# hcherkaoui/pybold

Measured on AMD Instinct MI355X. Metric: voxel-iterations/sec, higher is better.
Workload: dtype f16x2-split operands (22 bit), f32 accumulate, f64 iterate

## Files before the change

include/pybold_hip.h:

```cpp
#ifndef PYBOLD_HIP_H
#define PYBOLD_HIP_H

#include <stdint.h>

#ifdef __cplusplus
extern "C" {
#endif

#define PB_OK 0
#define PB_ERR_INVALID (-1)
#define PB_ERR_HIP (-2)

#define PB_FLAG_FORCE_GENERIC 1u
#define PB_FLAG_FORCE_FAST 2u
#define PB_FLAG_NO_PAIR 4u
#define PB_FLAG_FORCE_PAIR 8u
#define PB_FLAG_FORCE_WIDE 16u
#define PB_FLAG_DIRECT_FIR 64u
#define PB_FLAG_ONE_STREAM 128u
#define PB_FLAG_COLD_START 256u
#define PB_FLAG_NO_CERT 512u
#define PB_FLAG_CERT_NO_RESOLVE 2048u
#define PB_FLAG_FORCE_MFMA 16384u
#define PB_FLAG_NO_RHO_GUARD 32768u
#define PB_FLAG_FORCE_MFMA2 65536u
#define PB_FLAG_NO_MFMA 8192u
#define PB_FLAG_FORCE_CERT 1024u
#define PB_FLAG_NO_PARTITION 4096u
#define PB_FLAG_ONLY_DENSE 131072u
#define PB_FLAG_ONLY_SPARSE 262144u
#define PB_FLAG_NO_ILL_GUARD 524288u
#define PB_FLAG_PP_SPLIT 1048576u
#define PB_FLAG_LONG_HRF 2097152u
enum { PB_FLAG_MFMA_DENSE_TILES = 4194304 };
enum { PB_FLAG_GROUPED_SPLIT = 8388608 };
#define PB_FLAG_ONE_LAUNCH 32u

#define PB_STOP_NONE 0
#define PB_STOP_LOOPS 1
#define PB_STOP_WINDOW 2

int pb_version(void);

int pb_init(void);

const char* pb_last_error(void);

int pb_fista_has_fast_path(int N, int K);

int pb_fista_which_kernel(int N, int K, int P, int with_cost_trace, int stop_mode, int wind);

int pb_fista_plan(int N, int K, int P, int stop_mode, int wind, int* n_main, int* main_form,
                  int* tail_form);
int pb_fista_plan_ex(int N, int K, int P, int stop_mode, int wind, unsigned flags, int* n_main,
                     int* main_form, int* tail_form);

int pb_fista_solve(const float* y_dev, int64_t ldy, int y_rep,
                   double* w_dev, int64_t ldw, int P, int N,
                   const double* taps_host, const double* taps_dev, int K,
                   double step, double lbda, const double* lbda_dev,
                   const double* betas_dev, int n_iter,
                   float* J_dev, int64_t ldj,
                   int stop_mode, double tol, int wind, int32_t* n_done_dev,
                   unsigned flags, void* stream);

int64_t pb_fista_work_len(int P, int y_rep);
#define PB_CAND_COUNT 10
int pb_fista_list_plan(int kind, int n, int n_max, int has_pair, int has_wide, int one_stream, int has_mfma2,
// ... 222 lines not shown
```

pybold_amd/_lib.py:

```python
import ctypes
import os

_HERE = os.path.dirname(os.path.abspath(__file__))
LIB_PATH = os.environ.get("PYBOLD_HIP_LIB") or os.path.join(_HERE, "libpybold_hip.so")

PB_FLAG_FORCE_GENERIC = 1
PB_FLAG_FORCE_FAST = 2
PB_FLAG_NO_PAIR = 4
PB_FLAG_FORCE_PAIR = 8
PB_FLAG_FORCE_WIDE = 16
PB_FLAG_ONE_LAUNCH = 32
PB_FLAG_DIRECT_FIR = 64
PB_FLAG_ONE_STREAM = 128
PB_FLAG_COLD_START = 256
PB_FLAG_NO_CERT = 512
PB_FLAG_FORCE_CERT = 1024
PB_FLAG_CERT_NO_RESOLVE = 2048
PB_FLAG_NO_PARTITION = 4096
PB_FLAG_NO_MFMA = 8192
PB_FLAG_FORCE_MFMA = 16384
PB_FLAG_NO_RHO_GUARD = 32768
PB_FLAG_FORCE_MFMA2 = 65536
PB_FLAG_ONLY_DENSE = 131072
PB_FLAG_ONLY_SPARSE = 262144
PB_FLAG_NO_ILL_GUARD = 524288
PB_FLAG_PP_SPLIT = 1048576
PB_FLAG_MFMA_DENSE_TILES = 4194304
PB_FLAG_LONG_HRF = 2097152
PB_FLAG_GROUPED_SPLIT = 8388608
PB_PATH_DENSE_RATIO = 0.19
PB_STOP_NONE = 0
PB_STOP_LOOPS = 1
PB_STOP_WINDOW = 2

_c_int = ctypes.c_int
_c_i64 = ctypes.c_int64
_c_dbl = ctypes.c_double
_ptr = ctypes.c_void_p

_SOLVE_D = [
    _ptr, _c_i64, _c_int,
    _ptr, _c_i64, _c_int, _c_int,
    _ptr, _ptr, _c_int,
    _c_dbl, _c_dbl, _ptr,
    _ptr, _c_int,
    _ptr, _c_i64,
    _c_int, _c_dbl, _c_int, _ptr,
    ctypes.c_uint, _ptr]
_SOLVE_PP_D = [
    _ptr, _c_i64, _c_int,
    _ptr, _c_i64, _c_int, _c_int,
    _ptr, _c_i64, _c_int, _ptr,
    _c_dbl, _ptr,
    _ptr, _c_int,
    _ptr, _c_i64,
    _c_int, _c_dbl, _c_int, _ptr,
    ctypes.c_uint, _ptr]
_AUTO_LBDA_D = [
    _ptr, _c_i64, _ptr, _c_i64, _c_int, _c_int, _c_int,
    _ptr, _c_int, _c_dbl, _ptr, _ptr,
    _c_int, _c_dbl, _c_int, _c_int, _c_int, _c_int,
    _ptr, _ptr, _ptr, _c_i64,
# ... 176 lines not shown
```

pybold_amd/csrc/capi.hip:

```cpp
#include "../../include/pybold_hip.h"

#include <cstdarg>
#include <cstdlib>
#include <cstdio>
#include <cmath>
#include <cstring>
#include <map>
#include <mutex>

#include "fista_fast.h"
#include "generic.h"
#include "launch_fast.h"
#include "fista_pair.h"
#include "fista_pair_ffa.h"
#include "fista_exact.h"
#include "fista_exact_split.h"
#include "fista_auto.h"
#include "fista_exact_pp.h"
#include "fista_exact_split_pp.h"
#include "blind.h"
#include "fista_mfma.h"
#include "fista_mfma_sparse.h"
#include "fista_mfma_grouped.h"
#include "grouped.h"
#include "fista_mfma2.h"
#include "fista_mfma4.h"
#include "fista_mfma_split_grouped.h"
#include "path.h"
#include "dispatch.h"

namespace {

thread_local char g_err[512] = "";

int fail(int code, const char* fmt, ...) {
  va_list ap;
  va_start(ap, fmt);
  vsnprintf(g_err, sizeof(g_err), fmt, ap);
  va_end(ap);
  return code;
}

int check_launch(const char* what) {
  hipError_t e = hipGetLastError();
  if (e != hipSuccess) return fail(PB_ERR_HIP, "%s: %s", what, hipGetErrorString(e));
  g_err[0] = 0;
  return PB_OK;
}

constexpr int LDS_DOUBLES_MAX = 20000;
inline int64_t gen_lds_doubles(int N, int K, int stop_mode, int wind) {
  return 3 * (int64_t)N + K + 2 * pb::GEN_WAVES + (stop_mode == PB_STOP_WINDOW ? (int64_t)wind * N : 0);
}

inline int auto_outer_chunk(int form, int V, int nb_sub_iter) {
// ... 21 lines not shown
struct SideStream {
  hipStream_t stream = nullptr;
  hipEvent_t fork = nullptr, join = nullptr;
  bool ok = false;
};
std::mutex g_side_mutex;

SideStream* side_stream_locked() {
  static std::map<int, SideStream> per_dev;
  int dev = 0;
  if (hipGetDevice(&dev) != hipSuccess) return nullptr;
  SideStream& ss = per_dev[dev];
  if (!ss.ok && ss.stream == nullptr) {
    int least = 0, greatest = 0;
    if (hipDeviceGetStreamPriorityRange(&least, &greatest) != hipSuccess) { least = greatest = 0; (void)hipGetLastError(); }
    if (hipStreamCreateWithPriority(&ss.stream, hipStreamNonBlocking, greatest) == hipSuccess &&
        hipEventCreateWithFlags(&ss.fork, hipEventDisableTiming) == hipSuccess &&
        hipEventCreateWithFlags(&ss.join, hipEventDisableTiming) == hipSuccess)
      ss.ok = true;
    else
      (void)hipGetLastError();
  }
  return ss.ok ? &ss : nullptr;
}

bool stream_is_capturing(hipStream_t st) {
  hipStreamCaptureStatus cs = hipStreamCaptureStatusNone;
  if (hipStreamIsCapturing(st, &cs) != hipSuccess) {
    (void)hipGetLastError();
    return true;
  }
  return cs != hipStreamCaptureStatusNone;
}
struct WorkLayout { int64_t ranges, lmax, total; };
WorkLayout work_layout(int P, int V) {
  const int64_t nblk = ((int64_t)P + pb::PATH_PER_BLOCK - 1) / pb::PATH_PER_BLOCK;
  WorkLayout w;
  w.ranges = ((int64_t)P + 2 + 2 * nblk + 8 + 1) & ~(int64_t)1;
  w.lmax = w.ranges + 3 * 2 * pb::CAND_COUNT + 4;
  w.total = w.lmax + 2 * (int64_t)V + 8;
  return w;
}
int32_t* own_workspace(void* stream, int64_t need, int64_t* len) {
  static std::mutex mu;
  static std::map<std::pair<int, void*>, std::pair<int32_t*, int64_t>> cache;
  int dev = 0;
  if (hipGetDevice(&dev) != hipSuccess) { (void)hipGetLastError(); return nullptr; }
  std::lock_guard<std::mutex> lock(mu);
  auto& e = cache[std::make_pair(dev, stream)];
  if (e.second < need) {
    int32_t* fresh = nullptr;
    const int64_t want = need + need / 4;
    if (hipMalloc((void**)&fresh, (size_t)want * sizeof(int32_t)) != hipSuccess) { (void)hipGetLastError(); return nullptr; }
    e.first = fresh;
    e.second = want;
  }
  *len = e.second;
  return e.first;
}

template <int KIND>
int launch_op(const double* x, int64_t ldx, double* out, int64_t ldo, int V, int n_src, int n_dst,
              const double* taps, int K, void* stream, const char* name) {
  if (V < 0 || n_src < 1 || n_dst < 1 || K < 0)
    return fail(PB_ERR_INVALID, "%s: bad size (V=%d n_src=%d n_dst=%d K=%d)", name, V, n_src, n_dst, K);
  if (ldx < n_src || ldo < n_dst) return fail(PB_ERR_INVALID, "%s: leading dimension too small", name);
  const int nmax = n_src > n_dst ? n_src : n_dst;
  if (2 * (int64_t)nmax + K + 8 > LDS_DOUBLES_MAX)
    return fail(PB_ERR_INVALID, "%s: row of %d with %d taps exceeds LDS", name, nmax, K);
  if (V == 0) return PB_OK;
  if (!x || !out || (K > 0 && !taps)) return fail(PB_ERR_INVALID, "%s: NULL pointer", name);
  const size_t lds = (size_t)(2 * nmax + K + 8) * sizeof(double);
// ... 278 lines not shown
}

struct PartitionSpecs { pb::PlanSpec dense, sparse, flagged; };
PartitionSpecs partition_specs(const Route& r, int N, bool one_stream) {
  const double slots = wave_slots();
  const int pair = r.has_pair ? 1 : 0, wide = r.has_wide ? 1 : 0, os = one_stream ? 1 : 0;
  if (r.path == PATH_PART_SHORT)
    return {{1, pair, wide, 0, os, r.has_mfma2 ? 1 : 0, r.beside_chunks, slots}, {2, pair, wide, 0, os, 0, 0, slots}, {2, 0, wide, 0, 1, 0, 0, slots}};
  PartitionSpecs s{{3, 0, 0, 0, 1, 1, 0, slots}, {4, pair, 0, 0, 1, 0, 0, slots}, {4, 0, 0, 0, 1, 0, 0, slots}};
  if (N > 640) {
    s.dense.pass_mult = 2;
    s.dense.rem_num16 = MFMA4_MIN_R_NUM;
  }
  s.dense.backup_form = s.sparse.backup_form = s.flagged.backup_form = r.backup_wide ? FORM_WIDE : FORM_FAST1;
  s.sparse.min_pair = SPLIT_MIN_P;
  return s;
}
bool list_has_form(const Route& r, int form, int list) {
  const bool lng = r.path == PATH_PART_LONG;
  if (form == FORM_MFMA) return list <= 1 && r.mfma != nullptr;
  if (form == FORM_MFMA2) return list <= 1 && (lng || r.has_mfma2);
  if (list == 1) return false;
  if (form == FORM_PAIR) return list != 3 && r.has_pair;
  if (form == FORM_WIDE) return lng ? r.backup_wide : r.has_wide;
  return !lng || !r.backup_wide;
}
int cand_bound(const Route& r, int c, int P) {
  if (r.path == PATH_PART_SHORT) return pb::cand_max_slots(c, P, wave_slots());
  return (c == pb::CAND_MFMA2 || c == pb::CAND_PAIR0 || c == pb::CAND_FAST0 || c == pb::CAND_WIDE) ? P : 0;
}

template <class LF>
int solve_list(const Route& r, const pb::FistaArgs& a, const LF& lf, hipStream_t user, Side& side, const int32_t* work_dev,
               const int32_t* ranges, int list, bool exact_rule) {
  pb::FistaArgs b = a;
  b.perm = work_dev;
  b.n_dense = work_dev + a.P;
  b.perm_side = list == 3 ? 3 : 1;
  int rc = PB_OK;
  for (int c = 0; c < pb::CAND_COUNT && rc == PB_OK; ++c) {
    const int form = pb::cand_form(c);
    if (!list_has_form(r, form, list) || (pb::cand_side(c) && !side.ss)) continue;
    if ((c == pb::CAND_PAIR1 || c == pb::CAND_FAST1) && !side.ss) continue;
    b.grid_slots = cand_bound(r, c, a.P);
    if (b.grid_slots <= 0) continue;
    if (c >= pb::CAND_FIRST_AFTER_FORK && side.ss) rc = side.fork(user, lf.name);
    if (rc != PB_OK) break;
    b.range = ranges + 2 * c;
    rc = launch(lf, form, b, (pb::cand_side(c) && side.ss) ? side.ss->stream : user, exact_rule);
  }
  const int rj = side.join(user, lf.name);
  return rj != PB_OK ? rj : rc;
}

void launch_lmax_pass(const pb::FistaArgs& a, int V_series, const double* taps_host, double* lm, double gamma_f64, double gamma_vec,
                      hipStream_t st) {
  const int N = a.N, K = a.K;
  pb::LmaxTaps lt;
  double run = 0.0, csum = 0.0;
  for (int k = 0; k < pb::LMAX_KT; ++k) lt.h[k] = k < K ? (float)taps_host[k] : 0.0f;
  for (int t = 0; t < N; ++t) { if (t < K) run += taps_host[t]; csum += std::fabs(run); }
  const double unit = csum / std::sqrt((double)N);
  const float f64_bound = gamma_f64 > 0.0 ? (float)(gamma_f64 * unit) : 0.0f, vec_bound = gamma_vec > 0.0 ? (float)(gamma_vec * unit) : 0.0f;
  const dim3 grid((unsigned)((V_series + 3) / 4)), block(256);
  if (N <= 320) hipLaunchKernelGGL((pb::lmax_wave_kernel<5>), grid, block, 4 * (64 * 5 + pb::LMAX_KT) * sizeof(float), st, a.y, a.ldy, V_series, N, lt, K, lm, f64_bound, vec_bound);
  else if (N <= 640) hipLaunchKernelGGL((pb::lmax_wave_kernel<10>), grid, block, 4 * (64 * 10 + pb::LMAX_KT) * sizeof(float), st, a.y, a.ldy, V_series, N, lt, K, lm, f64_bound, vec_bound);
  else hipLaunchKernelGGL((pb::lmax_wave_kernel<21>), grid, block, 4 * (64 * 21 + pb::LMAX_KT) * sizeof(float), st, a.y, a.ldy, V_series, N, lt, K, lm, f64_bound, vec_bound);
}

int launch_partition(const pb::ClassPred& cp, int P, int32_t* work_dev, const pb::PlanSpec& front, const pb::PlanSpec& back,
                     int32_t* rg_front, int32_t* rg_back, int32_t* rg_ill, const char* what, hipStream_t st) {
  const int nblk = (P + pb::PATH_PER_BLOCK - 1) / pb::PATH_PER_BLOCK;
  hipLaunchKernelGGL(pb::path_count_kernel, dim3(nblk), dim3(pb::PATH_THREADS), 0, st, cp, P, work_dev);
  hipLaunchKernelGGL(pb::path_scan_kernel, dim3(1), dim3(pb::PATH_THREADS), 0, st, P, nblk, work_dev, front, back, rg_front, rg_back, rg_ill);
  hipLaunchKernelGGL(pb::path_scatter_kernel, dim3(nblk), dim3(pb::PATH_THREADS), 0, st, cp, P, work_dev);
  return check_launch(what);
}

void launch_generic(const pb::FistaArgs& a, const double* taps_dev, int K, int wind, bool with_j, bool f64, int grid, hipStream_t st) {
  void (*const kernel)(pb::FistaArgs, const double*, int, int) =
      !f64 ? (with_j ? pb::fista_generic_kernel<true> : pb::fista_generic_kernel<false>)
           : (with_j ? pb::fista_generic_kernel<true, true> : pb::fista_generic_kernel<false, true>);
  hipLaunchKernelGGL(kernel, dim3(grid), dim3(pb::GEN_THREADS), (size_t)gen_lds_doubles(a.N, K, a.stop_mode, wind) * sizeof(double), st,
                     a, taps_dev, K, wind);
}

template <class LF>
int run_partition(const Route& r, const pb::FistaArgs& a, const LF& lf, hipStream_t user, const double* taps_host,
                  const double* taps_dev, unsigned flags, double dense_ratio, int32_t* work_dev) {
  const int P = a.P, N = a.N, K = a.K, V_series = (P + a.y_rep - 1) / a.y_rep;
  const bool one_stream = r.path == PATH_PART_LONG || (flags & PB_FLAG_ONE_STREAM) != 0 || stream_is_capturing(user);
  const PartitionSpecs sp = partition_specs(r, N, one_stream);
  const WorkLayout wl = work_layout(P, V_series);
  const ExactEntry* ill_exact = pick_f64_default(N, K, a.stop_mode, a.wind, true);
  const bool ill_generic = !ill_exact && taps_dev && gen_lds_doubles(N, K, a.stop_mode, a.wind) <= LDS_DOUBLES_MAX;
  const bool guard = !(flags & PB_FLAG_NO_ILL_GUARD);
  double* lmax = reinterpret_cast<double*>(work_dev + wl.lmax);
  launch_lmax_pass(a, V_series, taps_host, lmax, (guard && (ill_exact || ill_generic)) ? PART_GAMMA_F64 : 0.0,
                   guard ? part_gamma_matrix_pipe(N, K) : 0.0, user);
  int32_t* rg_dense = work_dev + wl.ranges;
  int32_t* rg_sparse = rg_dense + 2 * pb::CAND_COUNT;
  int32_t* rg_flag = rg_sparse + 2 * pb::CAND_COUNT;
  int32_t* rg_ill = rg_flag + 2 * pb::CAND_COUNT;
  const double ratio = (r.path == PATH_PART_SHORT && !r.mfma) ? 0.0
                       : dense_ratio > 0.0 ? dense_ratio
                       : N > 640 ? PB_PATH_DENSE_RATIO_LONGER : (N > MFMA1_NMAX ? PB_PATH_DENSE_RATIO_LONG : PB_PATH_DENSE_RATIO);
  pb::PlanSpec front = sp.dense;
  front.merged = 1;
  int rc = launch_partition(pb::ClassPred{a.lbda_vec, a.lbda, lmax, a.y_rep, ratio, nullptr}, P, work_dev, front, sp.sparse, rg_dense,
                            rg_sparse, rg_ill, "partition", user);
  if (rc != PB_OK) return rc;
  Side side;
  if (!one_stream) side.take();
  const bool only_dense = (flags & PB_FLAG_ONLY_DENSE) != 0, only_sparse = (flags & PB_FLAG_ONLY_SPARSE) != 0;
  rc = solve_list(r, a, lf, user, side, work_dev, rg_dense, only_dense ? 1 : (only_sparse ? 2 : 0), false);
  if (rc != PB_OK || only_dense || only_sparse) return rc;
  if (ill_exact || ill_generic) {
    pb::FistaArgs b = a;
    b.perm = work_dev;
    b.perm_side = 1;
    b.range = rg_ill;
    if (ill_exact) {
      b.grid_slots = P;
      if (ill_exact->fn(b, taps_host, K, a.J != nullptr, a.stop_mode, user) != 0)
        return fail(PB_ERR_INVALID, "%s: float64 kernel rejected the launch (ill-conditioned series)", lf.name);
    } else {
      launch_generic(b, taps_dev, K, a.wind, a.J != nullptr, false, P < 2048 ? P : 2048, user);
    }
    rc = check_launch("float64 kernel (ill-conditioned series)");
    if (rc != PB_OK) return rc;
  }
  const pb::PlanSpec none{0, 0, 0, 0, 1, 0, 0, sp.dense.slots};
  rc = launch_partition(pb::ClassPred{nullptr, 0.0, nullptr, 1, 0.0, a.n_done}, P, work_dev, sp.flagged, none, rg_flag, nullptr, nullptr,
                        "partition(handed back)", user);
  if (rc != PB_OK) return rc;
  side.ss = nullptr;
  return solve_list(r, a, lf, user, side, work_dev, rg_flag, 3, true);
}

int outputs_impl(const double* w_dev, int64_t ldw, int P, int N, const double* taps_dev, int64_t ldt, int K, double* z_dev,
                 int64_t ldz, double* x_dev, int64_t ldx, void* stream, bool pp, const char* name) {
  if (P < 0 || N < 1 || K < 1 || ldw < N || (pp && ldt < K) || (z_dev && ldz < N) || (x_dev && ldx < N))
    return fail(PB_ERR_INVALID, "%s: bad size", name);
  if (2 * (int64_t)N + K + 8 > LDS_DOUBLES_MAX) return fail(PB_ERR_INVALID, "%s: N=%d K=%d exceeds LDS", name, N, K);
  if (P == 0 || (!z_dev && !x_dev)) return PB_OK;
  if (!w_dev || !taps_dev) return fail(PB_ERR_INVALID, "%s: NULL pointer", name);
  const size_t lds = (size_t)(2 * N + K + 8) * sizeof(double);
  hipLaunchKernelGGL(pb::outputs_kernel, dim3(P), dim3(pb::GEN_THREADS), lds, (hipStream_t)stream,
// ... 68 lines not shown

static int solve_impl(const float* y_dev, int64_t ldy, int y_rep, double* w_dev, int64_t ldw, int P,
                      int N, const double* taps_host, const double* taps_dev, int K, double step,
                      double lbda,
                      const double* lbda_dev, const double* betas_dev, int n_iter, float* J_dev,
                      int64_t ldj, int stop_mode, double tol, int wind, int32_t* n_done_dev,
                      unsigned flags, void* stream, const double* lmax_dev, double dense_ratio,
                      int32_t* work_dev, int64_t work_len) {
  if (P < 0 || N < 1 || K < 1 || n_iter < 0 || y_rep < 1)
    return fail(PB_ERR_INVALID, "pb_fista_solve: bad size (P=%d N=%d K=%d n_iter=%d y_rep=%d)", P,
                N, K, n_iter, y_rep);
  if (P > 0 && (!y_dev || !w_dev || !taps_host || (n_iter > 0 && !betas_dev)))
    return fail(PB_ERR_INVALID, "pb_fista_solve: NULL pointer");
  if (P > (1 << 25)) return fail(PB_ERR_INVALID, "pb_fista_solve: more than 2^25 problems per launch");
  if (ldy < N || ldw < N) return fail(PB_ERR_INVALID, "pb_fista_solve: leading dimension < N");
  if (J_dev && ldj < n_iter) return fail(PB_ERR_INVALID, "pb_fista_solve: ldj < n_iter");
  if (!(step > 0.0)) return fail(PB_ERR_INVALID, "pb_fista_solve: step must be positive");
  if (!lbda_dev && lbda < 0.0) return fail(PB_ERR_INVALID, "pb_fista_solve: negative lbda (float64 entry point only)");
  if (stop_mode < PB_STOP_NONE || stop_mode > PB_STOP_WINDOW)
    return fail(PB_ERR_INVALID, "pb_fista_solve: unknown stop_mode %d", stop_mode);
  if (stop_mode == PB_STOP_WINDOW && wind < 2)
    return fail(PB_ERR_INVALID, "pb_fista_solve: wind must be >= 2");
  if (P == 0) return PB_OK;

  pb::FistaArgs a = fista_args(P, N, K, n_iter, y_rep, ldy, w_dev, ldw, step, lbda, lbda_dev, betas_dev, stop_mode, tol,
                               n_done_dev, flags);
  a.y = y_dev; a.J = J_dev; a.ldj = ldj; a.wind = wind;
#ifdef PB_DEVELOPMENT
  if (const char* yb = getenv("PB_MFMA_YBITS")) {
    const int v = atoi(yb);
    if (v >= 8 && v <= 15) a.ybits = v;
  }
#endif
  const int V_series = (P + y_rep - 1) / y_rep;
  const bool workspace = work_dev && work_len >= work_layout(P, V_series).total && !((flags & PB_FLAG_FORCE_MFMA) && !lmax_dev);
  const Route r = route(Call{N, K, P, stop_mode, wind, flags, J_dev != nullptr, lbda_dev != nullptr, n_done_dev != nullptr,
                             tol * (double)n_iter, taps_dev != nullptr, workspace, false});
  const hipStream_t user = (hipStream_t)stream;
  const HostTapsForms lf{r, "pb_fista_solve", taps_host, K, stop_mode, J_dev != nullptr, (flags & PB_FLAG_DIRECT_FIR) != 0};
  if (r.path == PATH_PART_LONG || r.path == PATH_PART_SHORT)
    return run_partition(r, a, lf, user, taps_host, taps_dev, flags, dense_ratio, work_dev);
  if (r.path != PATH_GENERIC) return run_in_place(r, a, lf, user, flags);
  if (flags & PB_FLAG_FORCE_FAST)
    return fail(PB_ERR_INVALID, "pb_fista_solve: no register-resident kernel for N=%d K=%d stop=%d",
                N, K, stop_mode);
  if (!taps_dev) return fail(PB_ERR_INVALID, "pb_fista_solve: taps_dev required for the generic kernel");
  if (gen_lds_doubles(N, K, stop_mode, wind) > LDS_DOUBLES_MAX)
    return fail(PB_ERR_INVALID, "pb_fista_solve: N=%d K=%d wind=%d exceeds LDS", N, K, wind);
  launch_generic(a, taps_dev, K, wind, J_dev != nullptr, false, P, user);
  return check_launch("fista_generic_kernel");
}

int pb_fista_list_plan(int kind, int n, int n_max, int has_pair, int has_wide, int one_stream, int has_mfma2,
                       int beside_chunks, int32_t* ranges, int32_t* bounds) {
  if (kind < 1 || kind > 3 || n < 0 || n_max < n) return fail(PB_ERR_INVALID, "pb_fista_list_plan: bad argument");
  Piece pc[pb::MAX_PIECES];
  int npc = 0;
  const double slots = wave_slots();
  if (n > 0 && kind == 1) npc = pb::plan_pieces_mfma(n, has_pair != 0, has_wide != 0, false, one_stream != 0, has_mfma2 != 0, beside_chunks, slots, pc);
  else if (n > 0 && kind == 2) npc = pb::plan_pieces(n, has_pair != 0, has_wide != 0, false, one_stream != 0, slots, pc);
  else if (kind == 3 && n_max > 0)
    npc = pb::plan_partitioned(n, n_max, has_pair != 0, has_wide != 0, one_stream != 0, has_mfma2 != 0, beside_chunks, slots, pc);
  int32_t rg[2 * pb::CAND_COUNT];
  const int rc = pb::plan_to_candidates(pc, npc, rg);
  for (int c = 0; c < pb::CAND_COUNT; ++c) {
    if (ranges) { ranges[2 * c] = rg[2 * c]; ranges[2 * c + 1] = rg[2 * c + 1]; }
// ... 806 lines not shown
```

pybold_amd/csrc/path.h:

```cpp
#pragma once
#include <hip/hip_runtime.h>
#include <stdint.h>

#include "plan.h"

namespace pb {

constexpr int PATH_THREADS = 256, PATH_PER_THREAD = 16, PATH_PER_BLOCK = PATH_THREADS * PATH_PER_THREAD;

struct ClassPred {
  const double* lbda;
  double lbda_s;
  const double* lmax;
  int y_rep;
  double ratio;
  const int32_t* n_done;
};

__device__ __forceinline__ int path_class(const ClassPred& c, int p) {
  if (c.n_done) return c.n_done[p] < 0 ? 0 : 1;
  const double lm = c.lmax[p / c.y_rep];
  if (lm < 0.0) return 2;
  const double lb = c.lbda ? c.lbda[p] : c.lbda_s;
  return lb < c.ratio * lm ? 0 : 1;
// ... 4 lines not shown
__global__ __launch_bounds__(PATH_THREADS) void path_count_kernel(ClassPred cp, int P, int32_t* work) {
  __shared__ int part[2][PATH_THREADS / 64];
  const int p0 = blockIdx.x * PATH_PER_BLOCK + threadIdx.x * PATH_PER_THREAD;
  int c = 0, ci = 0;
  for (int i = 0; i < PATH_PER_THREAD; ++i) {
    if (p0 + i >= P) break;
    const int k = path_class(cp, p0 + i);
    c += k == 0;
    ci += k == 2;
  }
  for (int o = 32; o > 0; o >>= 1) { c += __shfl_xor(c, o, 64); ci += __shfl_xor(ci, o, 64); }
  if ((threadIdx.x & 63) == 0) { part[0][threadIdx.x >> 6] = c; part[1][threadIdx.x >> 6] = ci; }
  __syncthreads();
  if (threadIdx.x == 0) {
    work[P + 1 + blockIdx.x] = part[0][0] + part[0][1] + part[0][2] + part[0][3];
    work[P + 1 + gridDim.x + blockIdx.x] = part[1][0] + part[1][1] + part[1][2] + part[1][3];
  }
}

struct PlanSpec {
  int kind;
  int has_pair, has_wide, one_launch, one_stream, has_mfma2, beside_chunks;
  double slots;
  int backup_form = FORM_WIDE;
  int min_pair = 1024;
  int pass_mult = 4;
  int rem_num16 = 5;
  int merged = 0;
};
__device__ __forceinline__ void plan_list(const PlanSpec& sp, int n, int32_t* ranges);
__device__ __forceinline__ void plan_call(const PlanSpec& front, const PlanSpec& back, int n_d, int P, int32_t* ranges);

__global__ __launch_bounds__(PATH_THREADS) void path_scan_kernel(int P, int nblk, int32_t* work, PlanSpec front, PlanSpec back,
                                                                  int32_t* ranges_front, int32_t* ranges_back, int32_t* range_ill) {
  __shared__ int buf[PATH_THREADS];
  __shared__ int carry;
  int total[2] = {0, 0};
  for (int which = 0; which < 2; ++which) {
    if (threadIdx.x == 0) carry = 0;
    __syncthreads();
    int32_t* cnt = work + P + 1 + which * nblk;
    for (int b0 = 0; b0 < nblk; b0 += PATH_THREADS) {
      const int b = b0 + (int)threadIdx.x;
      const int v = b < nblk ? cnt[b] : 0;
      buf[threadIdx.x] = v;
      __syncthreads();
      for (int o = 1; o < PATH_THREADS; o <<= 1) {
        const int add = threadIdx.x >= (unsigned)o ? buf[threadIdx.x - o] : 0;
        __syncthreads();
        buf[threadIdx.x] += add;
        __syncthreads();
      }
      if (b < nblk) cnt[b] = carry + buf[threadIdx.x] - v;
      __syncthreads();
      if (threadIdx.x == PATH_THREADS - 1) carry += buf[PATH_THREADS - 1];
      __syncthreads();
    }
    total[which] = carry;
    __syncthreads();
  }
  if (threadIdx.x == 0) {
    const int n_front = total[0], n_ill = total[1], P_eff = P - n_ill;
    work[P] = n_front;
    work[P + path_nill_offset(nblk)] = n_ill;
    if (range_ill) { range_ill[0] = P_eff; range_ill[1] = P; }
    if (ranges_front && front.merged) plan_call(front, back, n_front, P_eff, ranges_front);
    else {
      if (ranges_front) plan_list(front, n_front, ranges_front);
      if (ranges_back) plan_list(back, P_eff - n_front, ranges_back);
    }
  }
}

__global__ __launch_bounds__(PATH_THREADS) void path_scatter_kernel(ClassPred cp, int P, int32_t* work) {
  __shared__ int buf[2][PATH_THREADS];
  const int p0 = blockIdx.x * PATH_PER_BLOCK + threadIdx.x * PATH_PER_THREAD;
  unsigned mask = 0, maski = 0;
  int c = 0, ci = 0;
  for (int i = 0; i < PATH_PER_THREAD; ++i) {
    if (p0 + i >= P) break;
    const int k = path_class(cp, p0 + i);
    if (k == 0) { mask |= 1u << i; ++c; }
    if (k == 2) { maski |= 1u << i; ++ci; }
  }
  buf[0][threadIdx.x] = c;
  buf[1][threadIdx.x] = ci;
  __syncthreads();
  for (int o = 1; o < PATH_THREADS; o <<= 1) {
    const int add = threadIdx.x >= (unsigned)o ? buf[0][threadIdx.x - o] : 0;
    const int addi = threadIdx.x >= (unsigned)o ? buf[1][threadIdx.x - o] : 0;
    __syncthreads();
    buf[0][threadIdx.x] += add;
    buf[1][threadIdx.x] += addi;
    __syncthreads();
  }
  const int n_front = work[P];
  int d = work[P + 1 + blockIdx.x] + buf[0][threadIdx.x] - c;
  int e = work[P + 1 + gridDim.x + blockIdx.x] + buf[1][threadIdx.x] - ci;
  for (int i = 0; i < PATH_PER_THREAD; ++i) {
    const int p = p0 + i;
    if (p >= P) break;
    if (mask & (1u << i)) work[d++] = p;
    else if (maski & (1u << i)) work[P - 1 - (e++)] = p;
// ... 106 lines not shown
```

pybold_amd/csrc/plan.h:

```cpp
#pragma once
#include <hip/hip_runtime.h>
#include <stdint.h>

namespace pb {

#define PB_HD __host__ __device__ inline

enum Form { FORM_GENERIC = 0, FORM_FAST1 = 1, FORM_PAIR = 2, FORM_WIDE = 3, FORM_MFMA = 4, FORM_MFMA2 = 5, FORM_MFMA4 = 6 };

constexpr double COST_FAST1 = 0.63, COST_WIDE = 0.19, COST_PARTIAL = 0.56;
constexpr double COST_LAUNCH = 0.03, COST_LAUNCH_WIDE = 0.05;

PB_HD int problems_per_wave(int form) { return form == FORM_PAIR ? 8 : (form == FORM_FAST1 ? 4 : 1); }

PB_HD double form_cost(int form, int P, double slots) {
  const double unit = form == FORM_PAIR ? 1.0 : (form == FORM_FAST1 ? COST_FAST1 : COST_WIDE);
  const int ppw = problems_per_wave(form);
  const double r = (double)((P + ppw - 1) / ppw) / slots;
  const double whole = floor(r), part = r - whole;
  return (form == FORM_WIDE ? COST_LAUNCH_WIDE : COST_LAUNCH) +
         unit * (whole + (part == 0.0 ? 0.0 : (part <= 0.5 ? COST_PARTIAL : 1.0)));
}

PB_HD int best_form(int P, bool has_pair, bool has_wide, double slots, double* cost = nullptr) {
// ... 130 lines not shown
PB_HD int plan_partitioned(int n_d, int P, bool has_pair, bool has_wide, bool one_stream, bool has_mfma2, int beside_chunks,
                           double slots, Piece* out) {
  if (n_d >= P) return plan_pieces_mfma(P, has_pair, has_wide, false, one_stream, has_mfma2, beside_chunks, slots, out);
  int n = 0;
  const int round = (int)slots * 8;
  const int whole = (n_d / round) * round, R = n_d - whole;
  int covered = whole;
  if (R > round / 2) {
    covered = n_d;
    out[n++] = Piece{FORM_MFMA, 0, n_d, false, false};
  } else {
    if (whole > 0) out[n++] = Piece{FORM_MFMA, 0, whole, false, false};
    if (has_mfma2 && R > MFMA2_MIN_R) {
      out[n++] = Piece{FORM_MFMA2, whole, n_d, false, false};
      covered = n_d;
    }
  }
  Piece sub[4];
  const int m = plan_pieces(P - covered, has_pair, has_wide, false, one_stream, slots, sub);
  for (int i = 0; i < m; ++i) out[n++] = Piece{sub[i].form, sub[i].p0 + covered, sub[i].p1 + covered, sub[i].side, sub[i].group};
  return n;
}

enum Cand {
  CAND_MFMA = 0, CAND_PAIR0, CAND_FAST0, CAND_MFMA2, CAND_PAIR1, CAND_FAST1, CAND_WIDE,
  CAND_SIDE_WIDE0, CAND_SIDE_WIDE1, CAND_SIDE_FAST, CAND_COUNT
};
constexpr int CAND_FIRST_AFTER_FORK = CAND_MFMA2, CAND_FIRST_SIDE = CAND_SIDE_WIDE0;
PB_HD int cand_form(int c) {
  return c == CAND_MFMA ? FORM_MFMA : c == CAND_MFMA2 ? FORM_MFMA2 : (c == CAND_PAIR0 || c == CAND_PAIR1) ? FORM_PAIR
         : (c == CAND_FAST0 || c == CAND_FAST1 || c == CAND_SIDE_FAST) ? FORM_FAST1 : FORM_WIDE;
}
PB_HD bool cand_side(int c) { return c >= CAND_FIRST_SIDE; }

PB_HD int cand_max_slots(int c, int n_max, double slots) {
  const int round = (int)slots * 8;
  const int lim = c == CAND_MFMA || c == CAND_PAIR0 || c == CAND_FAST0 ? n_max
                  : c == CAND_MFMA2 ? round / 2
                  : c == CAND_PAIR1 || c == CAND_FAST1 || c == CAND_WIDE ? round
                  : c == CAND_SIDE_FAST ? round / 4
                  : (int)slots;
  return lim < n_max ? lim : n_max;
}

PB_HD int plan_to_candidates(const Piece* pc, int npc, int32_t* ranges) {
  for (int c = 0; c < 2 * CAND_COUNT; ++c) ranges[c] = 0;
  int rc = 0;
  for (int i = 0; i < npc; ++i) {
    if (pc[i].p1 <= pc[i].p0) continue;
    const auto taken = [&](int c) { return ranges[2 * c + 1] > ranges[2 * c]; };
    int c = -1;
    switch (pc[i].form) {
      case FORM_MFMA:  c = pc[i].side ? -1 : CAND_MFMA; break;
      case FORM_MFMA2: c = pc[i].side ? -1 : CAND_MFMA2; break;
      case FORM_PAIR:  c = pc[i].side ? -1 : ((pc[i].group || taken(CAND_PAIR0)) ? CAND_PAIR1 : CAND_PAIR0); break;
      case FORM_FAST1: c = pc[i].side ? CAND_SIDE_FAST : ((pc[i].group || taken(CAND_FAST0)) ? CAND_FAST1 : CAND_FAST0); break;
      case FORM_WIDE:  c = pc[i].side ? (taken(CAND_SIDE_WIDE0) ? CAND_SIDE_WIDE1 : CAND_SIDE_WIDE0) : CAND_WIDE; break;
      default: break;
    }
    if (c < 0) { rc = -1; continue; }
    if (!pc[i].side && !pc[i].group && (c == CAND_PAIR1 || c == CAND_FAST1)) {
      const int c0 = c == CAND_PAIR1 ? CAND_PAIR0 : CAND_FAST0;
      if (taken(c0) && ranges[2 * c0 + 1] == pc[i].p0) { ranges[2 * c0 + 1] = pc[i].p1; continue; }
    }
    if (taken(c)) { rc = -1; continue; }
    ranges[2 * c] = pc[i].p0;
// ... 53 lines not shown
```

pybold_amd/solver.py:

```python
import collections

import numpy as np
import torch

from . import _lib
from ._lib import (PB_FLAG_COLD_START, PB_FLAG_NO_CERT, PB_FLAG_FORCE_CERT, PB_FLAG_DIRECT_FIR, PB_FLAG_ONE_STREAM, PB_FLAG_FORCE_FAST, PB_FLAG_FORCE_GENERIC, PB_FLAG_FORCE_PAIR, PB_FLAG_FORCE_WIDE,
                   PB_FLAG_NO_PAIR, PB_FLAG_ONE_LAUNCH, PB_STOP_LOOPS, PB_STOP_NONE, PB_STOP_WINDOW)

_STOP = {None: PB_STOP_NONE, "none": PB_STOP_NONE, "loops": PB_STOP_LOOPS,
         "window": PB_STOP_WINDOW}
_FORCE = {None: 0, "generic": PB_FLAG_FORCE_GENERIC, "fast": PB_FLAG_FORCE_FAST,
          "fast1": PB_FLAG_FORCE_FAST | PB_FLAG_NO_PAIR | PB_FLAG_ONE_LAUNCH,
          "fast2": PB_FLAG_FORCE_FAST | PB_FLAG_FORCE_PAIR | PB_FLAG_ONE_LAUNCH,
          "fast2d": PB_FLAG_FORCE_FAST | PB_FLAG_FORCE_PAIR | PB_FLAG_ONE_LAUNCH | PB_FLAG_DIRECT_FIR,
          "direct": PB_FLAG_DIRECT_FIR,
          "wide": PB_FLAG_FORCE_FAST | PB_FLAG_FORCE_WIDE | PB_FLAG_ONE_LAUNCH,
          "one": PB_FLAG_ONE_LAUNCH, "seq": PB_FLAG_ONE_STREAM,
          "cert": PB_FLAG_FORCE_CERT, "cert2": PB_FLAG_FORCE_CERT | PB_FLAG_FORCE_PAIR | PB_FLAG_ONE_LAUNCH,
          "certonly": PB_FLAG_FORCE_CERT | PB_FLAG_FORCE_PAIR | PB_FLAG_ONE_LAUNCH | _lib.PB_FLAG_CERT_NO_RESOLVE,
          "nocert": PB_FLAG_NO_CERT,
          "valu": _lib.PB_FLAG_NO_MFMA, "valuseq": _lib.PB_FLAG_NO_MFMA | PB_FLAG_ONE_STREAM,
          "mfma": PB_FLAG_ONE_LAUNCH | _lib.PB_FLAG_FORCE_MFMA,
          "mfma_dense": PB_FLAG_ONE_LAUNCH | _lib.PB_FLAG_FORCE_MFMA | _lib.PB_FLAG_MFMA_DENSE_TILES,
          "dense_tiles": _lib.PB_FLAG_MFMA_DENSE_TILES,
          "mfma_denseonly": PB_FLAG_ONE_LAUNCH | _lib.PB_FLAG_FORCE_MFMA | _lib.PB_FLAG_MFMA_DENSE_TILES | _lib.PB_FLAG_CERT_NO_RESOLVE,
          "path_dense": _lib.PB_FLAG_ONLY_DENSE, "path_sparse": _lib.PB_FLAG_ONLY_SPARSE,
          "noill": _lib.PB_FLAG_NO_ILL_GUARD,
          "nopart": _lib.PB_FLAG_NO_PARTITION, "nopartseq": _lib.PB_FLAG_NO_PARTITION | PB_FLAG_ONE_STREAM,
          "mfma2": _lib.PB_FLAG_FORCE_MFMA2, "mfma2only": _lib.PB_FLAG_FORCE_MFMA2 | _lib.PB_FLAG_CERT_NO_RESOLVE,
          "mfma2cert": _lib.PB_FLAG_FORCE_MFMA2 | PB_FLAG_FORCE_CERT,
          "mfma2certonly": _lib.PB_FLAG_FORCE_MFMA2 | PB_FLAG_FORCE_CERT | _lib.PB_FLAG_CERT_NO_RESOLVE,
          "intermediate": _lib.PB_FLAG_NO_RHO_GUARD,
          "intermediate_noresolve": _lib.PB_FLAG_NO_RHO_GUARD | _lib.PB_FLAG_CERT_NO_RESOLVE,
          "noresolve": _lib.PB_FLAG_CERT_NO_RESOLVE,
          "mfmaonly": PB_FLAG_ONE_LAUNCH | _lib.PB_FLAG_FORCE_MFMA | _lib.PB_FLAG_CERT_NO_RESOLVE,
          "mfmacert": PB_FLAG_ONE_LAUNCH | _lib.PB_FLAG_FORCE_MFMA | PB_FLAG_FORCE_CERT,
          "mfmacertonly": PB_FLAG_ONE_LAUNCH | _lib.PB_FLAG_FORCE_MFMA | PB_FLAG_FORCE_CERT | _lib.PB_FLAG_CERT_NO_RESOLVE,
          "gsplit": _lib.PB_FLAG_GROUPED_SPLIT,
          "gsplit_mfma": PB_FLAG_ONE_LAUNCH | _lib.PB_FLAG_FORCE_MFMA | _lib.PB_FLAG_GROUPED_SPLIT,
          "gsplit_mfmaonly": PB_FLAG_ONE_LAUNCH | _lib.PB_FLAG_FORCE_MFMA | _lib.PB_FLAG_GROUPED_SPLIT | _lib.PB_FLAG_CERT_NO_RESOLVE}

_F64Names = collections.namedtuple("_F64Names", "search search_pp solve_query search_query")
_F64Form = collections.namedtuple("_F64Form", "key force solve solve_pp solve_query search_query search search_pp op public")
F64_FORMS = collections.OrderedDict((f.key, f) for f in (
    _F64Form("one_wave", "fast",
             ("pb_fista_solve_d", PB_FLAG_FORCE_FAST), ("pb_fista_solve_pp_d", PB_FLAG_FORCE_FAST),
             None, "pb_auto_lbda_supported", "pb_auto_lbda_d", "pb_auto_lbda_pp_d", "auto_lbda_solve",
             _F64Names("auto_lbda_solve", "auto_lbda_solve_pp", None, "auto_lbda_supported")),
    _F64Form("four_waves", "split",
             None, ("pb_fista_solve_pp_d", _lib.PB_FLAG_PP_SPLIT),
             "pb_fista_pp_split_supported", "pb_auto_lbda_split_supported", "pb_auto_lbda_split_d", "pb_auto_lbda_split_pp_d",
             "auto_lbda_solve_split",
             _F64Names("auto_lbda_solve_split", "auto_lbda_solve_split_pp", "pp_split_supported", "auto_lbda_split_supported")),
    _F64Form("long", "long_hrf",
             ("pb_fista_solve_d", _lib.PB_FLAG_LONG_HRF), ("pb_fista_solve_pp_d", _lib.PB_FLAG_LONG_HRF),
             "pb_fista_long_hrf_supported", "pb_auto_lbda_long_supported", "pb_auto_lbda_long_d", "pb_auto_lbda_long_pp_d",
             "auto_lbda_solve_long",
             _F64Names("auto_lbda_solve_long", "auto_lbda_solve_long_pp", "long_hrf_supported", "auto_lbda_long_supported")),
    _F64Form("four_waves_long", "split_long_hrf",
             ("pb_fista_solve_split_long_d", 0), ("pb_fista_solve_split_long_pp_d", 0),
             "pb_fista_split_long_hrf_supported", "pb_auto_lbda_split_long_supported", "pb_auto_lbda_split_long_d",
             "pb_auto_lbda_split_long_pp_d", "auto_lbda_solve_split_long",
             _F64Names("auto_lbda_solve_split_long", "auto_lbda_solve_split_long_pp", "split_long_hrf_supported",
                       "auto_lbda_split_long_supported"))))
_F64_BY_FORCE = dict((f.force, f) for f in F64_FORMS.values())
_F64_SPLIT_PP_ONLY = "force='split' names the four-wave form with one HRF per problem: fista_solve_pp_d only"
_F64_FORCE_NAMES = {
    False: "float64 y: force must be None, 'fast' (register-resident float64 "
           "kernel, one problem per wave), 'generic' (LDS kernel), 'long_hrf' (the register form "
           "for HRFs of up to 48 taps, up to 640 scans) or 'split_long_hrf' (the same over four waves, "
           "641..1280 scans)",
    True: "float64 y: force must be None, 'fast' (register-resident float64 kernel, one problem per "
          "wave), 'split' (the same over four waves, 641..1280 scans), 'generic' (LDS kernel), "
# ... 1087 lines not shown
```

Baseline: 4.712 billion.

## Route dense leftovers of wide candidates through a new MFMA row kernel

Adds a one-wave-per-voxel MFMA kernel that handles 129..320-sample series by applying the banded HRF operator as split-f16 matrix products, with DPP row shifts and a far-field correction. The partition scan now emits a split point for each wide candidate, so dense-classified voxels that previously fell to the vector wide kernel go to the MFMA row kernel, and only the remainder uses the vector path. The aim is to move this leftover work from VALU onto matrix cores. In exchange it adds an extra launch per wide candidate and depends on the split-precision guard falling back correctly.

After: 4.787 billion (median of 6 runs). 1.6% higher.

```diff
diff --git a/include/pybold_hip.h b/include/pybold_hip.h
--- a/include/pybold_hip.h
+++ b/include/pybold_hip.h
@@ -34,6 +34,7 @@
 #define PB_FLAG_LONG_HRF 2097152u
 enum { PB_FLAG_MFMA_DENSE_TILES = 4194304 };
 enum { PB_FLAG_GROUPED_SPLIT = 8388608 };
+enum { PB_FLAG_VECTOR_LEFTOVERS = 16777216, PB_FLAG_FORCE_MFMA_ROW = 33554432 };
 #define PB_FLAG_ONE_LAUNCH 32u
 
 #define PB_STOP_NONE 0
diff --git a/pybold_amd/_lib.py b/pybold_amd/_lib.py
--- a/pybold_amd/_lib.py
+++ b/pybold_amd/_lib.py
@@ -28,6 +28,8 @@
 PB_FLAG_MFMA_DENSE_TILES = 4194304
 PB_FLAG_LONG_HRF = 2097152
 PB_FLAG_GROUPED_SPLIT = 8388608
+PB_FLAG_VECTOR_LEFTOVERS = 16777216
+PB_FLAG_FORCE_MFMA_ROW = 33554432
 PB_PATH_DENSE_RATIO = 0.19
 PB_STOP_NONE = 0
 PB_STOP_LOOPS = 1
diff --git a/pybold_amd/csrc/capi.hip b/pybold_amd/csrc/capi.hip
--- a/pybold_amd/csrc/capi.hip
+++ b/pybold_amd/csrc/capi.hip
@@ -21,6 +21,7 @@
 #include "blind.h"
 #include "fista_mfma.h"
 #include "fista_mfma_sparse.h"
+#include "fista_mfma_row.h"
 #include "fista_mfma_grouped.h"
 #include "grouped.h"
 #include "fista_mfma2.h"
@@ -108,12 +109,13 @@
   }
   return cs != hipStreamCaptureStatusNone;
 }
-struct WorkLayout { int64_t ranges, lmax, total; };
+struct WorkLayout { int64_t ranges, split, lmax, total; };
 WorkLayout work_layout(int P, int V) {
   const int64_t nblk = ((int64_t)P + pb::PATH_PER_BLOCK - 1) / pb::PATH_PER_BLOCK;
   WorkLayout w;
   w.ranges = ((int64_t)P + 2 + 2 * nblk + 8 + 1) & ~(int64_t)1;
-  w.lmax = w.ranges + 3 * 2 * pb::CAND_COUNT + 4;
+  w.split = w.ranges + 3 * 2 * pb::CAND_COUNT + 4;
+  w.lmax = w.split + 3 * pb::WIDE_CANDS + 3;
   w.total = w.lmax + 2 * (int64_t)V + 8;
   return w;
 }
@@ -458,7 +460,7 @@
 
 template <class LF>
 int solve_list(const Route& r, const pb::FistaArgs& a, const LF& lf, hipStream_t user, Side& side, const int32_t* work_dev,
-               const int32_t* ranges, int list, bool exact_rule) {
+               const int32_t* ranges, int list, bool exact_rule, const int32_t* split = nullptr, const double* taps_host = nullptr) {
   pb::FistaArgs b = a;
   b.perm = work_dev;
   b.n_dense = work_dev + a.P;
@@ -473,7 +475,17 @@
     if (c >= pb::CAND_FIRST_AFTER_FORK && side.ss) rc = side.fork(user, lf.name);
     if (rc != PB_OK) break;
     b.range = ranges + 2 * c;
-    rc = launch(lf, form, b, (pb::cand_side(c) && side.ss) ? side.ss->stream : user, exact_rule);
+    const hipStream_t st = (pb::cand_side(c) && side.ss) ? side.ss->stream : user;
+    if (split && form == FORM_WIDE) {
+      const int32_t* cut = split + 3 * pb::wide_cand_index(c);
+      b.range = cut;
+      rc = pb::launch_mfma_row(b, taps_host, a.K, false, st) != 0
+               ? fail(PB_ERR_INVALID, "%s: fista_mfma_row_kernel rejected its launch", lf.name)
+               : check_launch("fista_mfma_row_kernel");
+      if (rc != PB_OK) break;
+      b.range = cut + 1;
+    }
+    rc = launch(lf, form, b, st, exact_rule);
   }
   const int rj = side.join(user, lf.name);
   return rj != PB_OK ? rj : rc;
@@ -495,10 +507,10 @@
 }
 
 int launch_partition(const pb::ClassPred& cp, int P, int32_t* work_dev, const pb::PlanSpec& front, const pb::PlanSpec& back,
-                     int32_t* rg_front, int32_t* rg_back, int32_t* rg_ill, const char* what, hipStream_t st) {
+                     int32_t* rg_front, int32_t* rg_back, int32_t* rg_ill, const char* what, hipStream_t st, int32_t* rg_split = nullptr) {
   const int nblk = (P + pb::PATH_PER_BLOCK - 1) / pb::PATH_PER_BLOCK;
   hipLaunchKernelGGL(pb::path_count_kernel, dim3(nblk), dim3(pb::PATH_THREADS), 0, st, cp, P, work_dev);
-  hipLaunchKernelGGL(pb::path_scan_kernel, dim3(1), dim3(pb::PATH_THREADS), 0, st, P, nblk, work_dev, front, back, rg_front, rg_back, rg_ill);
+  hipLaunchKernelGGL(pb::path_scan_kernel, dim3(1), dim3(pb::PATH_THREADS), 0, st, P, nblk, work_dev, front, back, rg_front, rg_back, rg_ill, rg_split);
   hipLaunchKernelGGL(pb::path_scatter_kernel, dim3(nblk), dim3(pb::PATH_THREADS), 0, st, cp, P, work_dev);
   return check_launch(what);
 }
@@ -533,13 +545,18 @@
                        : N > 640 ? PB_PATH_DENSE_RATIO_LONGER : (N > MFMA1_NMAX ? PB_PATH_DENSE_RATIO_LONG : PB_PATH_DENSE_RATIO);
   pb::PlanSpec front = sp.dense;
   front.merged = 1;
+  const bool row_leftovers = r.path == PATH_PART_SHORT && r.mfma && !(flags & PB_FLAG_VECTOR_LEFTOVERS) && taps_host &&
+                             N >= pb::ROW_NMIN && N <= pb::ROW_NMAX && K <= pb::ROW_KMAX && a.stop_mode == PB_STOP_NONE && !a.J &&
+                             !a.taps_pp && a.n_done;
+  int32_t* rg_split = row_leftovers ? work_dev + wl.split : nullptr;
   int rc = launch_partition(pb::ClassPred{a.lbda_vec, a.lbda, lmax, a.y_rep, ratio, nullptr}, P, work_dev, front, sp.sparse, rg_dense,
-                            rg_sparse, rg_ill, "partition", user);
+                            rg_sparse, rg_ill, "partition", user, rg_split);
   if (rc != PB_OK) return rc;
   Side side;
   if (!one_stream) side.take();
   const bool only_dense = (flags & PB_FLAG_ONLY_DENSE) != 0, only_sparse = (flags & PB_FLAG_ONLY_SPARSE) != 0;
-  rc = solve_list(r, a, lf, user, side, work_dev, rg_dense, only_dense ? 1 : (only_sparse ? 2 : 0), false);
+  rc = solve_list(r, a, lf, user, side, work_dev, rg_dense, only_dense ? 1 : (only_sparse ? 2 : 0), false,
+                  (only_dense || only_sparse) ? nullptr : rg_split, taps_host);
   if (rc != PB_OK || only_dense || only_sparse) return rc;
   if (ill_exact || ill_generic) {
     pb::FistaArgs b = a;
@@ -674,6 +691,14 @@
     if (v >= 8 && v <= 15) a.ybits = v;
   }
 #endif
+  if (flags & PB_FLAG_FORCE_MFMA_ROW) {
+    if (N < pb::ROW_NMIN || N > pb::ROW_NMAX || K > pb::ROW_KMAX || J_dev || stop_mode != PB_STOP_NONE || !n_done_dev)
+      return fail(PB_ERR_INVALID, "pb_fista_solve: PB_FLAG_FORCE_MFMA_ROW serves plain solves of %d .. %d scans with up to %d taps, "
+                  "no cost trace, n_done_dev given (N=%d K=%d stop=%d)", pb::ROW_NMIN, pb::ROW_NMAX, pb::ROW_KMAX, N, K, stop_mode);
+    if (pb::launch_mfma_row(a, taps_host, K, false, (hipStream_t)stream) != 0)
+      return fail(PB_ERR_INVALID, "pb_fista_solve: fista_mfma_row_kernel rejected its launch");
+    return check_launch("fista_mfma_row_kernel");
+  }
   const int V_series = (P + y_rep - 1) / y_rep;
   const bool workspace = work_dev && work_len >= work_layout(P, V_series).total && !((flags & PB_FLAG_FORCE_MFMA) && !lmax_dev);
   const Route r = route(Call{N, K, P, stop_mode, wind, flags, J_dev != nullptr, lbda_dev != nullptr, n_done_dev != nullptr,
diff --git a/pybold_amd/csrc/fista_mfma_row.h b/pybold_amd/csrc/fista_mfma_row.h
--- /dev/null
+++ b/pybold_amd/csrc/fista_mfma_row.h
@@ -0,0 +1,228 @@
+#pragma once
+#include "mfma_core.h"
+
+namespace pb {
+
+constexpr int ROW_NMIN = 129, ROW_NMAX = 320, ROW_KMAX = 33;
+
+int launch_mfma_row(const FistaArgs& a, const double* taps, int K, bool with_j, hipStream_t st);
+
+#ifdef PB_MFMA_ROW_INST
+
+__device__ __forceinline__ unsigned row_word_from_below(unsigned v) {
+  return (unsigned)__builtin_amdgcn_update_dpp(0, (int)v, DPP_ROW_SHR + 1, 0xf, 0xf, true);
+}
+__device__ __forceinline__ unsigned row_word_from_above(unsigned v) {
+  return (unsigned)__builtin_amdgcn_update_dpp(0, (int)v, DPP_ROW_SHL + 1, 0xf, 0xf, true);
+}
+template <bool UP>
+__device__ __forceinline__ Frag row_neighbour(const u4& h, const u4& l) {
+  u4 nh, nl;
+#pragma unroll
+  for (int c = 0; c < 4; ++c) {
+    nh[c] = UP ? row_word_from_below(h[c]) : row_word_from_above(h[c]);
+    nl[c] = UP ? row_word_from_below(l[c]) : row_word_from_above(l[c]);
+  }
+  return Frag{__builtin_bit_cast(h8, nh), __builtin_bit_cast(h8, nl)};
+}
+__device__ __forceinline__ float column_sum(float x) {
+  float a = x, b = x;
+  asm("s_nop 1\n\tv_permlane32_swap_b32 %0, %1" : "+v"(a), "+v"(b));
+  a += b;
+  b = a;
+  asm("s_nop 1\n\tv_permlane16_swap_b32 %0, %1" : "+v"(a), "+v"(b));
+  return a + b;
+}
+__device__ __forceinline__ float wave_max(float x, int lane) {
+#pragma unroll
+  for (int o = 1; o < 64; o <<= 1)
+    x = fmaxf(x, __builtin_bit_cast(float, __builtin_amdgcn_ds_bpermute((lane ^ o) << 2, __builtin_bit_cast(int, x))));
+  return x;
+}
+
+__global__ __launch_bounds__(256) __attribute__((amdgpu_waves_per_eu(4, 4))) void fista_mfma_row_kernel(FistaArgs a, MfmaTaps tp) {
+  const int lane = threadIdx.x & 63, wv = threadIdx.x >> 6;
+  const int n = lane & 15, g = lane >> 4;
+  int s0 = 0, n_list = 0;
+  launch_slots(a, s0, n_list);
+  const int slot = __builtin_amdgcn_readfirstlane((int)blockIdx.x * 4 + wv) + s0;
+  if (slot >= n_list) return;
+  bool live;
+  const int p = __builtin_amdgcn_readfirstlane(slot_to_problem(a, slot, n_list, live));
+
+  __shared__ float lc_wg[4][64];
+  __shared__ f4 lys_wg[4][2][64];
+  float* lc = lc_wg[wv];
+  f4 (*lys)[64] = lys_wg[wv];
+  lc[lane] = tp.c[lane];
+  wave_sync();
+  const float sfar = lc[63];
+
+  const int t0 = 32 * n + 8 * g;
+  const double lb = a.lbda_vec ? a.lbda_vec[p] : a.lbda;
+  float ysn[8];
+  double w[1][8];
+  float sigma = 1.0f, inv_sigma = 1.0f;
+  bool degenerate = false;
+  {
+    const float* yrow = a.y + (int64_t)(p / a.y_rep) * a.ldy;
+    float m = 0.0f;
+#pragma unroll
+    for (int j = 0; j < 8; ++j) {
+      const int t = t0 + j;
+      float yl = yrow[t < a.N ? t : a.N - 1];
+      ysn[j] = t < a.N ? yl : 0.0f;
+      m = fmaxf(m, fabsf(ysn[j]));
+    }
+    m = __builtin_bit_cast(float, __builtin_amdgcn_readfirstlane(__builtin_bit_cast(int, wave_max(m, lane))));
+    const bool okm = m > 0.0f && m < 3.0e38f;
+    int e = 0;
+    (void)frexpf(okm ? m : 1.0f, &e);
+    e = __builtin_amdgcn_readfirstlane(e);
+    const float sg = ldexpf(1.0f, a.ybits - e) / tp.y_scale, isg = ldexpf(1.0f, e - a.ybits) * tp.y_scale;
+    sigma = okm ? sg : 1.0f;
+    inv_sigma = okm ? isg : 1.0f;
+    degenerate = !okm && !a.cold;
+    const float ys = -sigma * tp.y_scale;
+    const double* wrow = a.w + (int64_t)p * a.ldw;
+#pragma unroll
+    for (int j = 0; j < 8; ++j) {
+      ysn[j] *= ys;
+      w[0][j] = 0.0;
+    }
+#pragma unroll
+    for (int r = 0; r < 2; ++r) lys[r][lane] = f4{ysn[4 * r], ysn[4 * r + 1], ysn[4 * r + 2], ysn[4 * r + 3]};
+    if (!a.cold) {
+#pragma unroll
+      for (int j = 0; j < 8; ++j) {
+        const int t = t0 + j;
+        const double wl = wrow[t < a.N ? t : a.N - 1] * (double)sigma;
+        w[0][j] = t < a.N ? wl : 0.0;
+      }
+    }
+  }
+  const double th = lb * a.step * (double)sigma;
+  const double nstep = -a.step * tp.g_scale;
+  const int nvalid = a.N - t0;
+  __builtin_amdgcn_sched_barrier(0);
+  Frag An[2][2], Bn[2][2];
+  {
+    const int rho = lane & 15, kg = lane >> 4, gp = rho >> 2, i = rho & 3;
+    auto cval = [&](int lag) -> float {
+      const float c = lc[lag < 0 ? 0 : (lag > 63 ? 63 : lag)];
+      return lag < 0 ? 0.0f : c;
+    };
+#pragma unroll
+    for (int r = 0; r < 2; ++r)
+#pragma unroll
+      for (int o = 0; o < 2; ++o) {
+        float fa[8], fb[8];
+#pragma unroll
+        for (int j = 0; j < 8; ++j) {
+          const int ko = 8 * gp + 4 * r + i, ki = 8 * kg + j;
+          fa[j] = cval(32 * o + ko - ki);
+          fb[j] = cval(32 * o + ki - ko);
+        }
+        An[r][o] = split8(fa);
+        Bn[r][o] = split8(fb);
+        __builtin_amdgcn_sched_barrier(0);
+      }
+  }
+
+  float wmax = 0.0f, rmax = 0.0f;
+  double dummy0 = 0.0, dummy1 = 0.0;
+
+  for (int it = 0; it < a.n_iter; ++it) {
+    const double nb1 = -(1.0 + a.betas[it]);
+    float x[8];
+    u4 ph, pl;
+#pragma unroll
+    for (int j = 0; j < 8; ++j) {
+      x[j] = (float)w[0][j];
+      wmax = fmaxf(wmax, fabsf(x[j]));
+    }
+#pragma unroll
+    for (int pp = 0; pp < 4; ++pp) {
+      unsigned h2, l2;
+      (void)split_pair(x[2 * pp], x[2 * pp + 1], h2, l2);
+      ph[pp] = h2;
+      pl[pp] = l2;
+    }
+    const float fsum = column_sum(((x[0] + x[1]) + (x[2] + x[3])) + ((x[4] + x[5]) + (x[6] + x[7])));
+    const Frag wf{__builtin_bit_cast(h8, ph), __builtin_bit_cast(h8, pl)};
+    const Frag wf1 = row_neighbour<true>(ph, pl);
+    f4 acc[2];
+#pragma unroll
+    for (int r = 0; r < 2; ++r) acc[r] = lys[r][lane];
+#pragma unroll
+    for (int k = 0; k < 3; ++k)
+#pragma unroll
+      for (int r = 0; r < 2; ++r) acc[r] = mfma_part(An[r][0], wf, acc[r], k);
+#pragma unroll
+    for (int k = 0; k < 3; ++k)
+#pragma unroll
+      for (int r = 0; r < 2; ++r) acc[r] = mfma_part(An[r][1], wf1, acc[r], k);
+    {
+      const float far = sfar * row_from_below<2>(row_prefix_incl(fsum));
+#pragma unroll
+      for (int j = 0; j < 8; ++j) {
+        const float rj = acc[j >> 2][j & 3] + far;
+        x[j] = j < nvalid ? rj : 0.0f;
+        rmax = fmaxf(rmax, fabsf(x[j]));
+      }
+    }
+#pragma unroll
+    for (int pp = 0; pp < 4; ++pp) {
+      unsigned h2, l2;
+      (void)split_pair(x[2 * pp], x[2 * pp + 1], h2, l2);
+      ph[pp] = h2;
+      pl[pp] = l2;
+    }
+    const float bsum = column_sum(((x[0] + x[1]) + (x[2] + x[3])) + ((x[4] + x[5]) + (x[6] + x[7])));
+    const Frag rf{__builtin_bit_cast(h8, ph), __builtin_bit_cast(h8, pl)};
+    const Frag rf1 = row_neighbour<false>(ph, pl);
+#pragma unroll
+    for (int r = 0; r < 2; ++r) acc[r] = mfma_part(Bn[r][0], rf, f4{0.f, 0.f, 0.f, 0.f}, 0);
+#pragma unroll
+    for (int k = 1; k < 3; ++k)
+#pragma unroll
+      for (int r = 0; r < 2; ++r) acc[r] = mfma_part(Bn[r][0], rf, acc[r], k);
+#pragma unroll
+    for (int k = 0; k < 3; ++k)
+#pragma unroll
+      for (int r = 0; r < 2; ++r) acc[r] = mfma_part(Bn[r][1], rf1, acc[r], k);
+    {
+      const float far = sfar * row_from_above<2>(row_suffix_incl(bsum));
+#pragma unroll
+      for (int j = 0; j < 8; ++j)
+        (void)fista_update<false>(w[0][j], acc[j >> 2][j & 3] + far, nstep, th, nb1, dummy0, dummy1);
+    }
+  }
+
+  int le = threadIdx.x & 63;
+  asm volatile("" : "+v"(le));
+  const float wlast = wave_max(iterate_absmax<1>(w), le);
+  const float guard = wave_max(fmaxf(fmaxf(wmax, wlast), rmax >= 32768.0f ? 65504.0f : 0.0f), le);
+  const bool bad = !(guard < 60000.0f) || degenerate || (a.rho_guard && wlast > 0.0f && (float)th > MFMA_RHO_MAX * wlast);
+  if (live && !bad) {
+    const int te = 32 * (le & 15) + 8 * (le >> 4);
+    double* wrow = a.w + (int64_t)p * a.ldw + te;
+#pragma unroll
+    for (int j = 0; j < 8; ++j)
+      if (te + j < a.N) wrow[j] = w[0][j] * (double)inv_sigma;
+  }
+  if (live && a.n_done && lane == 0) a.n_done[p] = bad ? -1 : a.n_iter;
+}
+
+int launch_mfma_row(const FistaArgs& a, const double* taps, int K, bool with_j, hipStream_t st) {
+  if (a.N < ROW_NMIN || a.N > ROW_NMAX || K < 1 || K > ROW_KMAX) return 1;
+  if (with_j || a.stop_mode != 0 || a.taps_pp || a.only_flagged || !taps) return 1;
+  const int64_t waves = launch_count(a);
+  if (waves <= 0) return 0;
+  const MfmaTaps tp = make_mfma_taps(taps, K);
+  hipLaunchKernelGGL(fista_mfma_row_kernel, dim3((unsigned)((waves + 3) / 4)), dim3(256), 0, st, a, tp);
+  return 0;
+}
+#endif
+
+}
diff --git a/pybold_amd/csrc/mfma_row_inst.hip b/pybold_amd/csrc/mfma_row_inst.hip
--- /dev/null
+++ b/pybold_amd/csrc/mfma_row_inst.hip
@@ -0,0 +1,2 @@
+#define PB_MFMA_ROW_INST
+#include "fista_mfma_row.h"
diff --git a/pybold_amd/csrc/path.h b/pybold_amd/csrc/path.h
--- a/pybold_amd/csrc/path.h
+++ b/pybold_amd/csrc/path.h
@@ -60,7 +60,8 @@
 __device__ __forceinline__ void plan_call(const PlanSpec& front, const PlanSpec& back, int n_d, int P, int32_t* ranges);
 
 __global__ __launch_bounds__(PATH_THREADS) void path_scan_kernel(int P, int nblk, int32_t* work, PlanSpec front, PlanSpec back,
-                                                                  int32_t* ranges_front, int32_t* ranges_back, int32_t* range_ill) {
+                                                                  int32_t* ranges_front, int32_t* ranges_back, int32_t* range_ill,
+                                                                  int32_t* ranges_split = nullptr) {
   __shared__ int buf[PATH_THREADS];
   __shared__ int carry;
   int total[2] = {0, 0};
@@ -97,6 +98,15 @@
       if (ranges_front) plan_list(front, n_front, ranges_front);
       if (ranges_back) plan_list(back, P_eff - n_front, ranges_back);
     }
+    if (ranges_split && ranges_front) {
+      for (int k = 0; k < WIDE_CANDS; ++k) {
+        const int s0 = ranges_front[2 * wide_cand(k)], s1 = ranges_front[2 * wide_cand(k) + 1];
+        const int mid = n_front < s0 ? s0 : (n_front > s1 ? s1 : n_front);
+        ranges_split[3 * k] = s0;
+        ranges_split[3 * k + 1] = mid;
+        ranges_split[3 * k + 2] = s1;
+      }
+    }
   }
 }
 
diff --git a/pybold_amd/csrc/plan.h b/pybold_amd/csrc/plan.h
--- a/pybold_amd/csrc/plan.h
+++ b/pybold_amd/csrc/plan.h
@@ -186,6 +186,9 @@
          : (c == CAND_FAST0 || c == CAND_FAST1 || c == CAND_SIDE_FAST) ? FORM_FAST1 : FORM_WIDE;
 }
 PB_HD bool cand_side(int c) { return c >= CAND_FIRST_SIDE; }
+constexpr int WIDE_CANDS = 3;
+PB_HD int wide_cand(int k) { return k == 0 ? CAND_WIDE : (k == 1 ? CAND_SIDE_WIDE0 : CAND_SIDE_WIDE1); }
+PB_HD int wide_cand_index(int c) { return c == CAND_WIDE ? 0 : (c == CAND_SIDE_WIDE0 ? 1 : 2); }
 
 PB_HD int cand_max_slots(int c, int n_max, double slots) {
   const int round = (int)slots * 8;
diff --git a/pybold_amd/solver.py b/pybold_amd/solver.py
--- a/pybold_amd/solver.py
+++ b/pybold_amd/solver.py
@@ -38,7 +38,8 @@
           "mfmacertonly": PB_FLAG_ONE_LAUNCH | _lib.PB_FLAG_FORCE_MFMA | PB_FLAG_FORCE_CERT | _lib.PB_FLAG_CERT_NO_RESOLVE,
           "gsplit": _lib.PB_FLAG_GROUPED_SPLIT,
           "gsplit_mfma": PB_FLAG_ONE_LAUNCH | _lib.PB_FLAG_FORCE_MFMA | _lib.PB_FLAG_GROUPED_SPLIT,
-          "gsplit_mfmaonly": PB_FLAG_ONE_LAUNCH | _lib.PB_FLAG_FORCE_MFMA | _lib.PB_FLAG_GROUPED_SPLIT | _lib.PB_FLAG_CERT_NO_RESOLVE}
+          "gsplit_mfmaonly": PB_FLAG_ONE_LAUNCH | _lib.PB_FLAG_FORCE_MFMA | _lib.PB_FLAG_GROUPED_SPLIT | _lib.PB_FLAG_CERT_NO_RESOLVE,
+          "mfma_row": _lib.PB_FLAG_FORCE_MFMA_ROW, "vector_leftovers": _lib.PB_FLAG_VECTOR_LEFTOVERS}
 
 _F64Names = collections.namedtuple("_F64Names", "search search_pp solve_query search_query")
 _F64Form = collections.namedtuple("_F64Form", "key force solve solve_pp solve_query search_query search search_pp op public")
```
